# etzinis/sudo_rm_rf

Hardware: NVIDIA H100
Metric: mixtures_per_sec_forward_4s_8kHz_2src (higher is better)
Workload: dtype f32

## Files before the change

### sudo_rm_rf_b200/csrc/pointwise_mma.cu

```cuda
#include <cstdio>
#include <cstdlib>
#include <cstring>
#include <mutex>
#include <vector>
#include <cuda.h>
#include <cuda_bf16.h>
#include "common.cuh"

namespace sdr {

constexpr int kTileM = 128;
constexpr int kTileN = 128;
constexpr int kBlockK = 64;
constexpr int kStages = 3;
constexpr int kRawStages = 2;
constexpr int kBoxL = 32;
constexpr int kBoxBytes = 64 * kBoxL * 4;
constexpr int kRawStageBytes = kTileM / kBoxL * kBoxBytes;
constexpr int kBHalf = kTileN * 128;
constexpr int kBStageBytes = 2 * kBHalf;
constexpr int kSlotBytes = 2 * kBoxBytes;
constexpr int kSlots = 4;
constexpr int kConsWarps = 8, kTmaWarp = 8, kRawWarp = 9, kGatherWarps = 2;
template <bool WINDOW> constexpr int kMmaThreads = 32 * (kRawWarp + (WINDOW ? kGatherWarps : 1));

struct MmaArgs {
    const float* x;
    NormIn nin;
    const float* bias;
    int gate_channels;
    float* y;
    double* stats_out;
    int M, K, L;
    int l_tiles, n_tiles;
    int num_tiles;
    int epilogue;
    int win_k;
    int win_hop, win_pad, win_a;
    long long win_T;
};

__device__ __forceinline__ uint32_t smem_u32(const void* p) {
    return static_cast<uint32_t>(__cvta_generic_to_shared(p));
}
__device__ __forceinline__ void mbar_init(uint64_t* bar, uint32_t count) {
    asm volatile("mbarrier.init.shared::cta.b64 [%0], %1;" ::"r"(smem_u32(bar)), "r"(count) : "memory");
}
__device__ __forceinline__ void mbar_arrive(uint64_t* bar) {
    asm volatile("mbarrier.arrive.shared::cta.b64 _, [%0];" ::"r"(smem_u32(bar)) : "memory");
}
__device__ __forceinline__ void mbar_arrive_expect_tx(uint64_t* bar, uint32_t bytes) {
    asm volatile("mbarrier.arrive.expect_tx.shared::cta.b64 _, [%0], %1;" ::"r"(smem_u32(bar)), "r"(bytes) : "memory");
}
__device__ __forceinline__ void mbar_wait(uint64_t* bar, uint32_t parity) {
    const uint32_t addr = smem_u32(bar);
    uint32_t done;
    do {
        asm volatile(
            "{\n\t.reg .pred p;\n\t"
            "mbarrier.try_wait.parity.shared::cta.b64 p, [%1], %2;\n\t"
            "selp.u32 %0, 1, 0, p;\n\t}"
            : "=r"(done) : "r"(addr), "r"(parity) : "memory");
    } while (!done);
}
__device__ __forceinline__ void fence_barrier_init() {
    asm volatile("fence.mbarrier_init.release.cluster;" ::: "memory");
}
__device__ __forceinline__ void fence_proxy_async_smem() {
    asm volatile("fence.proxy.async.shared::cta;" ::: "memory");
}
__device__ __forceinline__ void tma_load_2d(void* smem_dst, const CUtensorMap* tm, uint64_t* bar, int c0, int c1) {
    asm volatile("cp.async.bulk.tensor.2d.shared::cluster.global.tile.mbarrier::complete_tx::bytes [%0], [%1, {%3, %4}], [%2];"
                 ::"r"(smem_u32(smem_dst)), "l"(tm), "r"(smem_u32(bar)), "r"(c0), "r"(c1) : "memory");
}
__device__ __forceinline__ void tma_load_3d(void* smem_dst, const CUtensorMap* tm, uint64_t* bar, int c0, int c1, int c2) {
    asm volatile("cp.async.bulk.tensor.3d.shared::cluster.global.tile.mbarrier::complete_tx::bytes [%0], [%1, {%3, %4, %5}], [%2];"
                 ::"r"(smem_u32(smem_dst)), "l"(tm), "r"(smem_u32(bar)), "r"(c0), "r"(c1), "r"(c2) : "memory");
}
__device__ __forceinline__ void tma_store_3d(const CUtensorMap* tm, const void* smem_src, int c0, int c1, int c2) {
    asm volatile("cp.async.bulk.tensor.3d.global.shared::cta.bulk_group [%0, {%2, %3, %4}], [%1];"
                 ::"l"(tm), "r"(smem_u32(smem_src)), "r"(c0), "r"(c1), "r"(c2) : "memory");
}
__device__ __forceinline__ void bulk_commit() { asm volatile("cp.async.bulk.commit_group;" ::: "memory"); }
__device__ __forceinline__ void bulk_wait_read_all() { asm volatile("cp.async.bulk.wait_group.read 0;" ::: "memory"); }
__device__ __forceinline__ void bulk_wait_all() { asm volatile("cp.async.bulk.wait_group 0;" ::: "memory"); }
__device__ __forceinline__ void named_bar_sync(uint32_t id, uint32_t threads) {
    asm volatile("bar.sync %0, %1;" ::"r"(id), "r"(threads) : "memory");
}

__device__ __forceinline__ uint64_t gmma_desc_sw128(uint32_t saddr, uint32_t lbo, uint32_t sbo) {
    uint64_t d = 0;
    d |= (uint64_t)((saddr >> 4) & 0x3FFF);
    d |= (uint64_t)((lbo >> 4) & 0x3FFF) << 16;
    d |= (uint64_t)((sbo >> 4) & 0x3FFF) << 32;
    d |= (uint64_t)1 << 62;
    return d;
}
constexpr uint32_t kBLbo = 16, kBSbo = 1024;

__device__ __forceinline__ void wgmma_fence() { asm volatile("wgmma.fence.sync.aligned;" ::: "memory"); }
__device__ __forceinline__ void wgmma_commit() { asm volatile("wgmma.commit_group.sync.aligned;" ::: "memory"); }
template <int N>
__device__ __forceinline__ void wgmma_wait() { asm volatile("wgmma.wait_group.sync.aligned %0;" ::"n"(N) : "memory"); }
__device__ __forceinline__ void wgmma_bf16_m64n128_rs(float (&d)[64], const uint32_t (&a)[4], uint64_t bdesc,
                                                      uint32_t accumulate) {
    asm volatile(
        "{\n\t.reg .pred p;\n\t"
        "setp.ne.b32 p, %69, 0;\n\t"
        "wgmma.mma_async.sync.aligned.m64n128k16.f32.bf16.bf16 "
        "{%0, %1, %2, %3, %4, %5, %6, %7, %8, %9, %10, %11, %12, %13, %14, %15, %16, %17, %18, %19, %20, %21, %22, "
        "%23, %24, %25, %26, %27, %28, %29, %30, %31, %32, %33, %34, %35, %36, %37, %38, %39, %40, %41, %42, %43, %44, "
        "%45, %46, %47, %48, %49, %50, %51, %52, %53, %54, %55, %56, %57, %58, %59, %60, %61, %62, %63}, "
        "{%64, %65, %66, %67}, %68, p, 1, 1, 0;\n\t}"
        : "+f"(d[0]), "+f"(d[1]), "+f"(d[2]), "+f"(d[3]), "+f"(d[4]), "+f"(d[5]), "+f"(d[6]), "+f"(d[7]),
          "+f"(d[8]), "+f"(d[9]), "+f"(d[10]), "+f"(d[11]), "+f"(d[12]), "+f"(d[13]), "+f"(d[14]), "+f"(d[15]),
          "+f"(d[16]), "+f"(d[17]), "+f"(d[18]), "+f"(d[19]), "+f"(d[20]), "+f"(d[21]), "+f"(d[22]), "+f"(d[23]),
          "+f"(d[24]), "+f"(d[25]), "+f"(d[26]), "+f"(d[27]), "+f"(d[28]), "+f"(d[29]), "+f"(d[30]), "+f"(d[31]),
          "+f"(d[32]), "+f"(d[33]), "+f"(d[34]), "+f"(d[35]), "+f"(d[36]), "+f"(d[37]), "+f"(d[38]), "+f"(d[39]),
          "+f"(d[40]), "+f"(d[41]), "+f"(d[42]), "+f"(d[43]), "+f"(d[44]), "+f"(d[45]), "+f"(d[46]), "+f"(d[47]),
          "+f"(d[48]), "+f"(d[49]), "+f"(d[50]), "+f"(d[51]), "+f"(d[52]), "+f"(d[53]), "+f"(d[54]), "+f"(d[55]),
          "+f"(d[56]), "+f"(d[57]), "+f"(d[58]), "+f"(d[59]), "+f"(d[60]), "+f"(d[61]), "+f"(d[62]), "+f"(d[63])
        : "r"(a[0]), "r"(a[1]), "r"(a[2]), "r"(a[3]), "l"(bdesc), "r"(accumulate)
        : "memory");
}

__global__ void pack_weight_mma_kernel(const float* __restrict__ W, uint8_t* __restrict__ out,
                                       int M, int Mpad, int Kreal, int K) {
    const long long i = (long long)blockIdx.x * blockDim.x + threadIdx.x;
    const long long chunks = (long long)Mpad * K / 8;
    if (i >= chunks) return;
    const int kc = (int)(i % (K / 8));
    const int m = (int)(i / (K / 8));
    const int kb = kc / 8, c = kc % 8;
    const int nt = m / kTileN, r = m % kTileN;
    const int KB = K / kBlockK;
    uint8_t* img = out + ((size_t)nt * KB + kb) * kBStageBytes;
    const size_t off = (size_t)(r >> 3) * 1024 + (size_t)(r & 7) * 128 + (size_t)((c ^ (r & 7)) << 4);
    __nv_bfloat16 hi[8], lo[8];
#pragma unroll
    for (int e = 0; e < 8; ++e) {
        const int k = kc * 8 + e;
        const float v = (m < M && k < Kreal) ? W[(size_t)m * Kreal + k] : 0.f;
        hi[e] = __float2bfloat16_rn(v);
        lo[e] = __float2bfloat16_rn(v - __bfloat162float(hi[e]));
    }
    *reinterpret_cast<uint4*>(img + off) = *reinterpret_cast<const uint4*>(hi);
    *reinterpret_cast<uint4*>(img + kBHalf + off) = *reinterpret_cast<const uint4*>(lo);
}

struct TileCoord { int sample, l0, n0; };
__device__ __forceinline__ TileCoord decode_tile(const MmaArgs& a, int tile) {
    TileCoord t;
    const int pos = tile / a.n_tiles;
    t.n0 = (tile - pos * a.n_tiles) * kTileN;
    t.sample = pos / a.l_tiles;
    t.l0 = (pos - t.sample * a.l_tiles) * kTileM;
    return t;
}

constexpr int kGroupSteps = 2;
constexpr int kGroups = kBlockK / 16 / kGroupSteps;
static_assert(kGroups == 2, "group g of every k-block uses fragment buffer g");
struct AFrag { uint32_t hi[kGroupSteps][4], lo[kGroupSteps][4]; };

template <bool WINDOW, int ACT, int MODE, bool STATS>
__global__ void __launch_bounds__(kMmaThreads<WINDOW>, 1)
pw_mma_kernel(const MmaArgs a, const __grid_constant__ CUtensorMap wmap,
              const __grid_constant__ CUtensorMap xmap,
              const __grid_constant__ CUtensorMap emap,
              const __grid_constant__ CUtensorMap ymap) {
    static_assert(!(WINDOW && ACT != 0), "the encoder's window operand has no activation");
    extern __shared__ uint8_t smem_raw[];
    uint8_t* smem = smem_raw + ((1024u - (smem_u32(smem_raw) & 1023u)) & 1023u);
    uint8_t* r_base = smem;
    uint8_t* b_base = r_base + kRawStages * kRawStageBytes;
    uint8_t* slots = b_base + kStages * kBStageBytes;
    float2* s_ab = reinterpret_cast<float2*>(slots + kSlots * kSlotBytes);
    float* s_sl = reinterpret_cast<float*>(s_ab + kRawStages * kBlockK);
    uint64_t* bars = reinterpret_cast<uint64_t*>(s_sl + kRawStages * kBlockK);
    uint64_t* full_bar = bars;
    uint64_t* empty_bar = full_bar + kStages;
    uint64_t* rfull_bar = empty_bar + kStages;
    uint64_t* rempty_bar = rfull_bar + kRawStages;
    uint64_t* slot_bar = rempty_bar + kRawStages;

    const int tid = threadIdx.x;
    const int warp = tid >> 5, lane = tid & 31;
    const int KB = a.K / kBlockK;
    const int tile0 = (int)blockIdx.x;
    const int tstep = (int)gridDim.x;

    if (warp == kTmaWarp && lane == 0) {
        for (int s = 0; s < kStages; ++s) { mbar_init(&full_bar[s], 1); mbar_init(&empty_bar[s], kConsWarps); }
        for (int s = 0; s < kRawStages; ++s) {
            mbar_init(&rfull_bar[s], WINDOW ? kGatherWarps : 2);
            mbar_init(&rempty_bar[s], kConsWarps);
        }
        for (int s = 0; s < kSlots; ++s) mbar_init(&slot_bar[s], 1);
        fence_barrier_init();
    }
    __syncthreads();

    if (warp >= kRawWarp) {
        int rs = 0;
        uint32_t rphase = 0;
        if constexpr (WINDOW) {
            constexpr int kGatherCh = kBlockK / kGatherWarps;
            const int c0 = (warp - kRawWarp) * kGatherCh;
#pragma unroll 1
            for (int tile = tile0; tile < a.num_tiles; tile += tstep) {
                const TileCoord tc = decode_tile(a, tile);
#pragma unroll 1
                for (int kb = 0; kb < KB; ++kb) {
                    uint8_t* rp = r_base + (size_t)rs * kRawStageBytes + (lane & 3) * 4;
#pragma unroll
                    for (int i0 = 0; i0 < kGatherCh; i0 += 16) {
                        float v[16][kTileM / kBoxL];
#pragma unroll
                        for (int i = 0; i < 16; ++i) {
                            const int k = kb * kBlockK + c0 + i0 + i;
                            const int ch = k / a.win_k, j = k - ch * a.win_k;
                            const float* src = a.x + ((size_t)tc.sample * a.win_a + ch) * a.win_T;
#pragma unroll
                            for (int b = 0; b < kTileM / kBoxL; ++b) {
                                const int l = tc.l0 + b * kBoxL + lane;
                                const long long t = (long long)a.win_hop * l + j - a.win_pad;
                                v[i][b] = (l < a.L && ch < a.win_a && t >= 0 && t < a.win_T) ? __ldg(src + t) : 0.f;
                            }
                        }
                        if (i0 == 0) mbar_wait(&rempty_bar[rs], rphase ^ 1);
#pragma unroll
                        for (int i = 0; i < 16; ++i) {
                            const int c = c0 + i0 + i;
#pragma unroll
                            for (int b = 0; b < kTileM / kBoxL; ++b)
                                *reinterpret_cast<float*>(rp + b * kBoxBytes + c * 128 + (((lane >> 2) ^ (c & 7)) << 4)) = v[i][b];
                        }
                    }
                    __syncwarp();
                    if (lane == 0) mbar_arrive(&rfull_bar[rs]);
                    if (++rs == kRawStages) { rs = 0; rphase ^= 1; }
                }
            }
        } else {
            const bool has_norm = a.nin.stats != nullptr;
            const double inv_count = 1.0 / a.nin.count;
#pragma unroll 1
            for (int tile = tile0; tile < a.num_tiles; tile += tstep) {
                const TileCoord tc = decode_tile(a, tile);
                float mean = 0.f, rstd = 1.f;
                if (has_norm) {
                    const double mu = a.nin.stats[2 * (size_t)tc.sample] * inv_count;
                    double var = a.nin.stats[2 * (size_t)tc.sample + 1] * inv_count - mu * mu;
                    var = var < 0.0 ? 0.0 : var;
                    mean = (float)mu;
                    rstd = rsqrtf((float)var + kGlnEps);
                }
#pragma unroll 1
                for (int kb = 0; kb < KB; ++kb) {
                    const int k = kb * kBlockK + 2 * lane;
                    float g[2] = {1.f, 1.f}, be[2] = {0.f, 0.f}, sl[2] = {1.f, 1.f};
                    if (has_norm) {
                        g[0] = __ldg(a.nin.gamma + k); g[1] = __ldg(a.nin.gamma + k + 1);
                        be[0] = __ldg(a.nin.beta + k); be[1] = __ldg(a.nin.beta + k + 1);
                    }
                    if constexpr (ACT == 2) { sl[0] = __ldg(a.nin.prelu + k); sl[1] = __ldg(a.nin.prelu + k + 1); }
                    mbar_wait(&rempty_bar[rs], rphase ^ 1);
                    if (lane == 0) {
                        mbar_arrive_expect_tx(&rfull_bar[rs], kRawStageBytes);
                        for (int b = 0; b < kTileM / kBoxL; ++b)
                            tma_load_3d(r_base + (size_t)rs * kRawStageBytes + b * kBoxBytes, &xmap, &rfull_bar[rs],
                                        tc.l0 + b * kBoxL, kb * kBlockK, tc.sample);
                    }
                    float aa[2] = {1.f, 1.f}, bb[2] = {0.f, 0.f};
                    if (has_norm) {
#pragma unroll
                        for (int e = 0; e < 2; ++e) { aa[e] = g[e] * rstd; bb[e] = be[e] - mean * aa[e]; }
                    }
                    *reinterpret_cast<float4*>(s_ab + rs * kBlockK + 2 * lane) = make_float4(aa[0], bb[0], aa[1], bb[1]);
                    if constexpr (ACT == 2) *reinterpret_cast<float2*>(s_sl + rs * kBlockK + 2 * lane) = make_float2(sl[0], sl[1]);
                    __syncwarp();
                    if (lane == 0) mbar_arrive(&rfull_bar[rs]);
                    if (++rs == kRawStages) { rs = 0; rphase ^= 1; }
                }
            }
        }
    } else if (warp == kTmaWarp) {
        if (lane == 0) {
            int stage = 0;
            uint32_t phase = 0;
            for (int tile = tile0; tile < a.num_tiles; tile += tstep) {
                const int nt = tile % a.n_tiles;
                for (int kb = 0; kb < KB; ++kb) {
                    mbar_wait(&empty_bar[stage], phase ^ 1);
                    mbar_arrive_expect_tx(&full_bar[stage], kBStageBytes);
                    tma_load_2d(b_base + (size_t)stage * kBStageBytes, &wmap, &full_bar[stage], 0, (nt * KB + kb) * 2 * kTileN);
                    if (++stage == kStages) { stage = 0; phase ^= 1; }
                }
            }
        }
        __syncwarp();
    } else {
        const int wg = warp >> 2;
        const int wr = warp & 3;
        const int q = lane & 3;
        const bool issuer = (tid & 127) == 0;
        const bool relu_out = WINDOW && a.epilogue == 2;
        const float slope = ACT == 1 ? __ldg(a.nin.prelu) : 1.f;
        const bool slope_le1 = slope <= 1.f;
        uint32_t boff[4];
#pragma unroll
        for (int v = 0; v < 4; ++v) {
            const uint32_t c = 2 * q + (v & 1), pp = 16 * (wr & 1) + (lane >> 2) + 8 * (v >> 1);
            boff[v] = c * 128 + (((pp >> 2) ^ c) << 4) + (pp & 3) * 4;
        }
        const uint32_t raw_box = (uint32_t)(2 * wg + (wr >> 1)) * kBoxBytes;
        uint8_t* const my_slots = slots + (size_t)(2 * wg) * kSlotBytes;
        auto fill_slot = [&](int tile, int h) {
            uint64_t* bar = &slot_bar[2 * wg + h];
            if constexpr (MODE == 0) {
                mbar_arrive(bar);
            } else {
                const TileCoord t = decode_tile(a, tile);
                const int c0 = t.l0 + 64 * wg;
                const int c1 = (MODE == 1 ? t.n0 : t.n0 % a.gate_channels) + 64 * h;
                uint8_t* const dst = my_slots + (size_t)h * kSlotBytes;
                mbar_arrive_expect_tx(bar, kSlotBytes);
                tma_load_3d(dst, &emap, bar, c0, c1, t.sample);
                tma_load_3d(dst + kBoxBytes, &emap, bar, c0 + kBoxL, c1, t.sample);
            }
        };
        if (issuer) { fill_slot(tile0, 0); fill_slot(tile0, 1); }

        int rs = 0, stage = 0, prev_stage = 0;
        uint32_t rphase = 0, phase = 0, slot_phase = 0;
        auto transform = [&](AFrag& f, int g) {
            if (g == 0) mbar_wait(&rfull_bar[rs], rphase);
            const uint8_t* rp = r_base + (size_t)rs * kRawStageBytes + raw_box;
            const float2* tab = s_ab + rs * kBlockK + 2 * q;
            const float* tsl = s_sl + rs * kBlockK + 2 * q;
#pragma unroll
            for (int s = 0; s < kGroupSteps; ++s) {
#pragma unroll
                for (int h = 0; h < 2; ++h) {
                    const int c = 16 * (g * kGroupSteps + s) + 8 * h;
                    float4 ab = make_float4(1.f, 0.f, 1.f, 0.f);
                    float2 sl = make_float2(1.f, 1.f);
                    if constexpr (!WINDOW) ab = *reinterpret_cast<const float4*>(tab + c);
                    if constexpr (ACT == 2) sl = *reinterpret_cast<const float2*>(tsl + c);
#pragma unroll
                    for (int ph = 0; ph < 2; ++ph) {
                        float y[2];
#pragma unroll
                        for (int e = 0; e < 2; ++e) {
                            const float x = *reinterpret_cast<const float*>(rp + boff[e + 2 * ph] + c * 128);
                            y[e] = WINDOW ? x : fmaf(x, e ? ab.z : ab.x, e ? ab.w : ab.y);
                            if constexpr (ACT == 1) {
                                const float t = y[e] * slope;
                                y[e] = slope_le1 ? fmaxf(y[e], t) : fminf(y[e], t);
                            } else if constexpr (ACT == 2) {
                                y[e] = y[e] >= 0.f ? y[e] : y[e] * (e ? sl.y : sl.x);
                            }
                        }
                        const uint32_t h0 = __float_as_uint(y[0]) & 0xffff0000u, h1 = __float_as_uint(y[1]) & 0xffff0000u;
                        const __nv_bfloat162 lo = __floats2bfloat162_rn(y[0] - __uint_as_float(h0), y[1] - __uint_as_float(h1));
                        f.hi[s][2 * h + ph] = __byte_perm(h0, h1, 0x7632);
                        f.lo[s][2 * h + ph] = *reinterpret_cast<const uint32_t*>(&lo);
                    }
                }
            }
            if (g == kGroups - 1) {
                __syncwarp();
                if (lane == 0) mbar_arrive(&rempty_bar[rs]);
                if (++rs == kRawStages) { rs = 0; rphase ^= 1; }
            }
        };
        float acc[64];
        auto mma_group = [&](int kb, int g, const AFrag& cur, AFrag& nxt) {
            if (g == 0) mbar_wait(&full_bar[stage], phase);
            const uint32_t sb_hi = smem_u32(b_base + (size_t)stage * kBStageBytes);
            const uint32_t sb_lo = sb_hi + kBHalf;
            wgmma_fence();
#pragma unroll
            for (int s = 0; s < kGroupSteps; ++s) {
                const int ks = g * kGroupSteps + s;
                const uint64_t dbh = gmma_desc_sw128(sb_hi + ks * 32, kBLbo, kBSbo);
                const uint64_t dbl = gmma_desc_sw128(sb_lo + ks * 32, kBLbo, kBSbo);
                wgmma_bf16_m64n128_rs(acc, cur.hi[s], dbh, (kb | ks) != 0 ? 1u : 0u);
                wgmma_bf16_m64n128_rs(acc, cur.lo[s], dbh, 1u);
                wgmma_bf16_m64n128_rs(acc, cur.hi[s], dbl, 1u);
            }
            wgmma_commit();
            wgmma_wait<1>();
            if (g == 0 && kb > 0) {
                __syncwarp();
                if (lane == 0) mbar_arrive(&empty_bar[prev_stage]);
            }
            if (g == kGroups - 1) {
                prev_stage = stage;
                if (++stage == kStages) { stage = 0; phase ^= 1; }
                if (kb + 1 < KB) transform(nxt, 0);
            } else {
                transform(nxt, g + 1);
            }
        };
        AFrag fa, fb;
#pragma unroll 1
        for (int tile = tile0; tile < a.num_tiles; tile += tstep) {
            const TileCoord tc = decode_tile(a, tile);
#pragma unroll
            for (int i = 0; i < 64; ++i) acc[i] = 0.f;
            transform(fa, 0);
#pragma unroll 1
            for (int kb = 0; kb < KB; ++kb) {
                mma_group(kb, 0, fa, fb);
                mma_group(kb, 1, fb, fa);
            }
            wgmma_wait<0>();
            __syncwarp();
            if (lane == 0) mbar_arrive(&empty_bar[prev_stage]);
            const int prem = a.L - (tc.l0 + wg * 64 + 32 * (wr >> 1) + 16 * (wr & 1) + (lane >> 2));
            StatAcc st;
            float rs_ = 0.f, rq = 0.f;
#pragma unroll
            for (int h = 0; h < 2; ++h) {
                uint8_t* const slot = my_slots + (size_t)h * kSlotBytes;
                uint8_t* const box = slot + (wr >> 1) * kBoxBytes;
                const int m0 = tc.n0 + 64 * h + 2 * q;
                const int mrem = a.M - m0;
                mbar_wait(&slot_bar[2 * wg + h], slot_phase);
#pragma unroll
                for (int j = 0; j < 8; ++j) {
                    float bv[2];
#pragma unroll
                    for (int b = 0; b < 2; ++b) bv[b] = (a.bias && 8 * j + b < mrem) ? __ldg(a.bias + m0 + 8 * j + b) : 0.f;
#pragma unroll
                    for (int v = 0; v < 4; ++v) {
                        const int u = 4 * j + v, i = 32 * h + u;
                        float* e = reinterpret_cast<float*>(box + boff[v] + 1024 * j);
                        float o = acc[i] + bv[v & 1];
                        if (MODE == 1) o += *e;
                        if (MODE == 2) o = fmaxf(o, 0.f) * *e;
                        if constexpr (WINDOW) { if (relu_out) o = fmaxf(o, 0.f); }
                        *e = o;
                        if (STATS && 8 * j + (v & 1) < mrem && 8 * (v >> 1) < prem) { rs_ += o; rq = fmaf(o, o, rq); }
                        if (STATS && (i & 15) == 15) { st.add_run(rs_, rq); rs_ = rq = 0.f; }
                    }
                }
                if constexpr (WINDOW) {
                    named_bar_sync(1 + wg, 128);
#pragma unroll 4
                    for (int r = wr; r < 64; r += 4) {
                        const int m = tc.n0 + 64 * h + r;
#pragma unroll
                        for (int half = 0; half < 2; ++half) {
                            const int p = tc.l0 + wg * 64 + half * kBoxL + lane;
                            const float v = *reinterpret_cast<const float*>(
                                slot + half * kBoxBytes + r * 128 + (((lane >> 2) ^ (r & 7)) << 4) + (lane & 3) * 4);
                            if (m < a.M && p < a.L) a.y[((size_t)tc.sample * a.M + m) * a.L + p] = v;
                        }
                    }
                    named_bar_sync(1 + wg, 128);
                } else {
                    fence_proxy_async_smem();
                    named_bar_sync(1 + wg, 128);
                    if (issuer) {
                        const int c0 = tc.l0 + wg * 64, c1 = tc.n0 + 64 * h;
                        tma_store_3d(&ymap, slot, c0, c1, tc.sample);
                        tma_store_3d(&ymap, slot + kBoxBytes, c0 + kBoxL, c1, tc.sample);
                        bulk_commit();
                        bulk_wait_read_all();
                    }
                }
                if (issuer && tile + tstep < a.num_tiles) fill_slot(tile + tstep, h);
            }
            slot_phase ^= 1;
            if (STATS) {
                const double ds = warp_sum_f64(st.s), dq = warp_sum_f64(st.q);
                if (lane == 0) {
                    atomicAdd(a.stats_out + 2 * (size_t)tc.sample, ds);
                    atomicAdd(a.stats_out + 2 * (size_t)tc.sample + 1, dq);
                }
            }
        }
        if (!WINDOW && issuer) bulk_wait_all();
    }
}

static inline int mma_pad_m(int M) { return (M + kTileN - 1) / kTileN * kTileN; }

bool pointwise_mma_eligible(int M, int K) {
    return M >= 32 && K >= kBlockK && (K % kBlockK) == 0;
}

size_t pointwise_mma_packed_bytes(int M, int K) {
    if (!pointwise_mma_eligible(M, K)) return 0;
    return (size_t)mma_pad_m(M) * K * 4;
}

int pack_pointwise_mma(const float* W, int M, int K, void* packed, cudaStream_t st) {
    if (!pointwise_mma_eligible(M, K)) return SDR_ERR_UNSUPPORTED;
    const int Mpad = mma_pad_m(M);
    const long long chunks = (long long)Mpad * K / 8;
    pack_weight_mma_kernel<<<(unsigned)((chunks + 255) / 256), 256, 0, st>>>(
        W, static_cast<uint8_t*>(packed), M, Mpad, K, K);
    return cudaGetLastError() == cudaSuccess ? SDR_OK : SDR_ERR_CUDA;
}

constexpr size_t kMmaSmemBytes = 1024 + (size_t)kRawStages * kRawStageBytes + (size_t)kStages * kBStageBytes +
                                 (size_t)kSlots * kSlotBytes + kRawStages * kBlockK * (sizeof(float2) + sizeof(float)) +
                                 (2 * kStages + 2 * kRawStages + kSlots) * sizeof(uint64_t);
static_assert(kMmaSmemBytes <= 232448, "exceeds the 227 KB a CTA may own on sm_90");

typedef CUresult (*EncodeTiledFn)(CUtensorMap*, CUtensorMapDataType, cuuint32_t, void*, const cuuint64_t*,
                                  const cuuint64_t*, const cuuint32_t*, const cuuint32_t*, CUtensorMapInterleave,
                                  CUtensorMapSwizzle, CUtensorMapL2promotion, CUtensorMapFloatOOBfill);
static EncodeTiledFn encode_tiled_fn() {
    static EncodeTiledFn fn = [] {
        void* ptr = nullptr;
        cudaDriverEntryPointQueryResult qres = cudaDriverEntryPointSymbolNotFound;
        if (cudaGetDriverEntryPoint("cuTensorMapEncodeTiled", &ptr, cudaEnableDefault, &qres) != cudaSuccess ||
            qres != cudaDriverEntryPointSuccess)
            ptr = nullptr;
        return reinterpret_cast<EncodeTiledFn>(ptr);
    }();
    return fn;
}

static int make_weight_map(CUtensorMap* tm, const void* wpk, size_t bytes) {
    memset(tm, 0, sizeof(*tm));
    EncodeTiledFn enc = encode_tiled_fn();
    if (!enc) return SDR_ERR_CUDA;
    const cuuint64_t dims[2] = {32, (cuuint64_t)(bytes / 128)};
    const cuuint64_t strides[1] = {128};
    const cuuint32_t box[2] = {32, (cuuint32_t)(2 * kTileN)};
    const cuuint32_t estr[2] = {1, 1};
    const CUresult r = enc(tm, CU_TENSOR_MAP_DATA_TYPE_FLOAT32, 2, const_cast<void*>(wpk), dims, strides, box, estr,
                           CU_TENSOR_MAP_INTERLEAVE_NONE, CU_TENSOR_MAP_SWIZZLE_NONE,
                           CU_TENSOR_MAP_L2_PROMOTION_L2_256B, CU_TENSOR_MAP_FLOAT_OOB_FILL_NONE);
    return r == CUDA_SUCCESS ? SDR_OK : SDR_ERR_UNSUPPORTED;
}

static int make_act_map(CUtensorMap* tm, const float* x, int samples, int C, int L) {
    memset(tm, 0, sizeof(*tm));
    EncodeTiledFn enc = encode_tiled_fn();
    if (!enc) return SDR_ERR_CUDA;
    const cuuint64_t dims[3] = {(cuuint64_t)L, (cuuint64_t)C, (cuuint64_t)samples};
    const cuuint64_t strides[2] = {(cuuint64_t)L * 4, (cuuint64_t)L * C * 4};
    const cuuint32_t box[3] = {(cuuint32_t)kBoxL, 64, 1};
    const cuuint32_t estr[3] = {1, 1, 1};
    const CUresult r = enc(tm, CU_TENSOR_MAP_DATA_TYPE_FLOAT32, 3, const_cast<float*>(x), dims, strides, box, estr,
                           CU_TENSOR_MAP_INTERLEAVE_NONE, CU_TENSOR_MAP_SWIZZLE_128B,
                           CU_TENSOR_MAP_L2_PROMOTION_L2_256B, CU_TENSOR_MAP_FLOAT_OOB_FILL_NONE);
    return r == CUDA_SUCCESS ? SDR_OK : SDR_ERR_UNSUPPORTED;
}
static_assert(kBlockK == 64 && kTileN == 2 * 64, "activation boxes are 64 channels: one k-block, half a channel tile");

struct MmaLaunchInfo { const void* fn; int dev; int sms; };
static std::mutex g_launch_mutex;
static std::vector<MmaLaunchInfo> g_launch_info;

template <bool WINDOW, typename Kern>
static int launch_persistent(Kern kern, const MmaArgs& a, const CUtensorMap& wmap, const CUtensorMap& xmap,
                             const CUtensorMap& emap, const CUtensorMap& ymap, cudaStream_t st) {
    int dev = 0;
    if (cudaGetDevice(&dev) != cudaSuccess) return SDR_ERR_CUDA;
    int sms = 0;
    {
        std::lock_guard<std::mutex> lock(g_launch_mutex);
        for (const MmaLaunchInfo& e : g_launch_info)
            if (e.fn == reinterpret_cast<const void*>(kern) && e.dev == dev) { sms = e.sms; break; }
        if (sms == 0) {
            if (cudaFuncSetAttribute(kern, cudaFuncAttributeMaxDynamicSharedMemorySize, (int)kMmaSmemBytes) != cudaSuccess) {
                cudaGetLastError();
                return SDR_ERR_CUDA;
            }
            if (cudaDeviceGetAttribute(&sms, cudaDevAttrMultiProcessorCount, dev) != cudaSuccess || sms <= 0) return SDR_ERR_CUDA;
            g_launch_info.push_back(MmaLaunchInfo{reinterpret_cast<const void*>(kern), dev, sms});
        }
    }
    const int grid = a.num_tiles < sms ? a.num_tiles : sms;
    kern<<<grid, kMmaThreads<WINDOW>, kMmaSmemBytes, st>>>(a, wmap, xmap, emap, ymap);
    if (cudaGetLastError() != cudaSuccess) return SDR_ERR_CUDA;
    return SDR_OK;
}

int launch_pointwise_mma(const float* x, const NormIn& nin, const void* wpk, const float* bias,
                         const float* residual, const float* gate, int gate_channels,
                         float* y, double* stats_out, int samples, int M, int K, int L,
                         int epilogue, cudaStream_t st) {
    auto misaligned = [](const float* p) { return (reinterpret_cast<uintptr_t>(p) % 16) != 0; };
    if (!pointwise_mma_eligible(M, K) || (L % 4) != 0 || misaligned(x) || misaligned(y) ||
        (epilogue != 1 && misaligned(residual)) || (epilogue == 1 && misaligned(gate)))
        return SDR_ERR_UNSUPPORTED;
    if (samples <= 0 || L <= 0 || !x || !wpk || !y) return SDR_ERR_BAD_ARGUMENT;
    if (epilogue == 1 && (!gate || gate_channels <= 0)) return SDR_ERR_BAD_ARGUMENT;
    if (epilogue == 1 && (gate_channels % kTileN) != 0) return SDR_ERR_UNSUPPORTED;
    if (reinterpret_cast<uintptr_t>(wpk) % 16) return SDR_ERR_BAD_ARGUMENT;
    MmaArgs a;
    a.x = x; a.nin = nin; a.bias = bias;
    a.gate_channels = gate_channels; a.y = y; a.stats_out = stats_out;
    a.M = M; a.K = K; a.L = L; a.epilogue = epilogue;
    a.win_k = 0; a.win_hop = 0; a.win_pad = 0; a.win_a = 0; a.win_T = 0;
    a.n_tiles = mma_pad_m(M) / kTileN;
    a.l_tiles = (L + kTileM - 1) / kTileM;
    const long long tiles = (long long)samples * a.l_tiles * a.n_tiles;
    if (tiles > 0x7fffffffLL) return SDR_ERR_UNSUPPORTED;
    a.num_tiles = (int)tiles;
    const int act = nin.prelu ? (nin.prelu_pc ? 2 : 1) : 0;
    const int mode = epilogue == 1 ? 2 : (residual ? 1 : 0);
    const bool stats = stats_out != nullptr;
    CUtensorMap wmap, xmap, emap, ymap;
    if (int rc = make_weight_map(&wmap, wpk, pointwise_mma_packed_bytes(M, K))) return rc;
    if (int rc = make_act_map(&xmap, x, samples, K, L)) return rc;
    if (int rc = make_act_map(&ymap, y, samples, M, L)) return rc;
    memset(&emap, 0, sizeof(emap));
    if (mode == 1)
        if (int rc = make_act_map(&emap, residual, samples, M, L)) return rc;
    if (mode == 2)
        if (int rc = make_act_map(&emap, gate, samples, gate_channels, L)) return rc;
#define SDR_MMA_CASE(A, MD, ST)                                                                                   \
    if (act == A && mode == MD && stats == ST)                                                                    \
        return launch_persistent<false>(pw_mma_kernel<false, A, MD, ST>, a, wmap, xmap, emap, ymap, st);
    SDR_MMA_CASE(0, 0, false) SDR_MMA_CASE(0, 0, true)
    SDR_MMA_CASE(1, 0, false) SDR_MMA_CASE(1, 0, true)
    SDR_MMA_CASE(0, 1, false) SDR_MMA_CASE(0, 1, true)
    SDR_MMA_CASE(1, 1, false) SDR_MMA_CASE(1, 1, true)
    SDR_MMA_CASE(0, 2, false) SDR_MMA_CASE(0, 2, true)
    SDR_MMA_CASE(1, 2, false) SDR_MMA_CASE(1, 2, true)
    SDR_MMA_CASE(2, 0, false) SDR_MMA_CASE(2, 0, true)
#undef SDR_MMA_CASE
    return SDR_ERR_UNSUPPORTED;
}

static inline int enc_kpad(int A, int Kk) { return (A * Kk + kBlockK - 1) / kBlockK * kBlockK; }

size_t encoder_mma_packed_bytes(int N, int A, int Kk) {
    if (N < 32 || A < 1 || Kk < 3) return 0;
    return (size_t)mma_pad_m(N) * enc_kpad(A, Kk) * 4;
}

int pack_encoder_mma(const float* W, int N, int A, int Kk, void* packed, cudaStream_t st) {
    if (!encoder_mma_packed_bytes(N, A, Kk)) return SDR_ERR_UNSUPPORTED;
    const int Mpad = mma_pad_m(N), K = enc_kpad(A, Kk);
    const long long chunks = (long long)Mpad * K / 8;
    pack_weight_mma_kernel<<<(unsigned)((chunks + 255) / 256), 256, 0, st>>>(
        W, static_cast<uint8_t*>(packed), N, Mpad, A * Kk, K);
    return cudaGetLastError() == cudaSuccess ? SDR_OK : SDR_ERR_CUDA;
}

int launch_encoder_mma(const float* wav, const void* wpk, const float* bias, int relu, float* enc, double* stats,
                       int B, int A, long long T, int N, int Kk, int L, int pad, cudaStream_t st) {
    if (!encoder_mma_packed_bytes(N, A, Kk)) return SDR_ERR_UNSUPPORTED;
    if (B <= 0 || T <= 0 || L <= 0 || !wav || !wpk || !enc) return SDR_ERR_BAD_ARGUMENT;
    MmaArgs a;
    a.x = wav; a.nin = NormIn{nullptr, nullptr, nullptr, nullptr, 1.0};
    a.bias = bias;
    a.gate_channels = 0; a.y = enc; a.stats_out = stats;
    a.M = N; a.K = enc_kpad(A, Kk); a.L = L; a.epilogue = relu ? 2 : 0;
    a.win_k = Kk; a.win_hop = Kk / 2; a.win_pad = pad; a.win_a = A; a.win_T = T;
    a.n_tiles = mma_pad_m(N) / kTileN;
    a.l_tiles = (L + kTileM - 1) / kTileM;
    const long long tiles = (long long)B * a.l_tiles * a.n_tiles;
    if (tiles > 0x7fffffffLL) return SDR_ERR_UNSUPPORTED;
    a.num_tiles = (int)tiles;
    CUtensorMap wmap, none;
    if (int rc = make_weight_map(&wmap, wpk, encoder_mma_packed_bytes(N, A, Kk))) return rc;
    memset(&none, 0, sizeof(none));
    if (stats) return launch_persistent<true>(pw_mma_kernel<true, 0, 0, true>, a, wmap, none, none, none, st);
    return launch_persistent<true>(pw_mma_kernel<true, 0, 0, false>, a, wmap, none, none, none, st);
}

}
```

Baseline: 2579.

## Move epilogue TMA stores and slot refills to a dedicated store warp

Adds a dedicated store warp for the non-window pointwise GEMM kernel. Consumer warpgroups now only arrive on a new per-slot full barrier, and the store warp issues the TMA stores, waits for the reads to finish, and refills the slot with residual or gate data for the next tile. This removes the named-barrier sync and the blocking bulk_wait_read from the consumer path, so math warps can move on to the next tile. The cost is one extra warp, extra mbarriers, and a single thread that serialises all four slots' stores and refills.

```diff
diff --git a/sudo_rm_rf_b200/csrc/pointwise_mma.cu b/sudo_rm_rf_b200/csrc/pointwise_mma.cu
--- a/sudo_rm_rf_b200/csrc/pointwise_mma.cu
+++ b/sudo_rm_rf_b200/csrc/pointwise_mma.cu
@@ -21,8 +21,9 @@
 constexpr int kBStageBytes = 2 * kBHalf;
 constexpr int kSlotBytes = 2 * kBoxBytes;
 constexpr int kSlots = 4;
-constexpr int kConsWarps = 8, kTmaWarp = 8, kRawWarp = 9, kGatherWarps = 2;
-template <bool WINDOW> constexpr int kMmaThreads = 32 * (kRawWarp + (WINDOW ? kGatherWarps : 1));
+constexpr int kConsWarps = 8, kTmaWarp = 8, kRawWarp = 9, kStoreWarp = 10, kGatherWarps = 2;
+constexpr int kMmaThreads = 32 * (kStoreWarp + 1);
+static_assert(kRawWarp + kGatherWarps == kStoreWarp + 1, "window mode's gather warps take the raw and store warps' places");
 
 struct MmaArgs {
     const float* x;
@@ -164,7 +165,7 @@
 struct AFrag { uint32_t hi[kGroupSteps][4], lo[kGroupSteps][4]; };
 
 template <bool WINDOW, int ACT, int MODE, bool STATS>
-__global__ void __launch_bounds__(kMmaThreads<WINDOW>, 1)
+__global__ void __launch_bounds__(kMmaThreads, 1)
 pw_mma_kernel(const MmaArgs a, const __grid_constant__ CUtensorMap wmap,
               const __grid_constant__ CUtensorMap xmap,
               const __grid_constant__ CUtensorMap emap,
@@ -183,6 +184,7 @@
     uint64_t* rfull_bar = empty_bar + kStages;
     uint64_t* rempty_bar = rfull_bar + kRawStages;
     uint64_t* slot_bar = rempty_bar + kRawStages;
+    uint64_t* slot_full = slot_bar + kSlots;
 
     const int tid = threadIdx.x;
     const int warp = tid >> 5, lane = tid & 31;
@@ -196,12 +198,12 @@
             mbar_init(&rfull_bar[s], WINDOW ? kGatherWarps : 2);
             mbar_init(&rempty_bar[s], kConsWarps);
         }
-        for (int s = 0; s < kSlots; ++s) mbar_init(&slot_bar[s], 1);
+        for (int s = 0; s < kSlots; ++s) { mbar_init(&slot_bar[s], 1); mbar_init(&slot_full[s], kConsWarps / 2); }
         fence_barrier_init();
     }
     __syncthreads();
 
-    if (warp >= kRawWarp) {
+    if (WINDOW ? warp >= kRawWarp : warp == kRawWarp) {
         int rs = 0;
         uint32_t rphase = 0;
         if constexpr (WINDOW) {
@@ -300,11 +302,49 @@
             }
         }
         __syncwarp();
+    } else if (warp == kStoreWarp) {
+        if constexpr (!WINDOW) {
+            if (lane == 0) {
+                auto fill_slot = [&](int tile, int s) {
+                    if constexpr (MODE == 0) {
+                        mbar_arrive(&slot_bar[s]);
+                    } else {
+                        const TileCoord t = decode_tile(a, tile);
+                        const int c0 = t.l0 + 64 * (s >> 1);
+                        const int c1 = (MODE == 1 ? t.n0 : t.n0 % a.gate_channels) + 64 * (s & 1);
+                        uint8_t* const dst = slots + (size_t)s * kSlotBytes;
+                        mbar_arrive_expect_tx(&slot_bar[s], kSlotBytes);
+                        tma_load_3d(dst, &emap, &slot_bar[s], c0, c1, t.sample);
+                        tma_load_3d(dst + kBoxBytes, &emap, &slot_bar[s], c0 + kBoxL, c1, t.sample);
+                    }
+                };
+                for (int s = 0; s < kSlots; ++s) fill_slot(tile0, s);
+                uint32_t phase = 0;
+#pragma unroll 1
+                for (int tile = tile0; tile < a.num_tiles; tile += tstep) {
+                    const TileCoord tc = decode_tile(a, tile);
+#pragma unroll 1
+                    for (int i = 0; i < kSlots; ++i) {
+                        const int h = i >> 1, wg = i & 1, s = 2 * wg + h;
+                        uint8_t* const slot = slots + (size_t)s * kSlotBytes;
+                        const int c0 = tc.l0 + 64 * wg, c1 = tc.n0 + 64 * h;
+                        mbar_wait(&slot_full[s], phase);
+                        tma_store_3d(&ymap, slot, c0, c1, tc.sample);
+                        tma_store_3d(&ymap, slot + kBoxBytes, c0 + kBoxL, c1, tc.sample);
+                        bulk_commit();
+                        bulk_wait_read_all();
+                        if (tile + tstep < a.num_tiles) fill_slot(tile + tstep, s);
+                    }
+                    phase ^= 1;
+                }
+                bulk_wait_all();
+            }
+            __syncwarp();
+        }
     } else {
         const int wg = warp >> 2;
         const int wr = warp & 3;
         const int q = lane & 3;
-        const bool issuer = (tid & 127) == 0;
         const bool relu_out = WINDOW && a.epilogue == 2;
         const float slope = ACT == 1 ? __ldg(a.nin.prelu) : 1.f;
         const bool slope_le1 = slope <= 1.f;
@@ -316,21 +356,6 @@
         }
         const uint32_t raw_box = (uint32_t)(2 * wg + (wr >> 1)) * kBoxBytes;
         uint8_t* const my_slots = slots + (size_t)(2 * wg) * kSlotBytes;
-        auto fill_slot = [&](int tile, int h) {
-            uint64_t* bar = &slot_bar[2 * wg + h];
-            if constexpr (MODE == 0) {
-                mbar_arrive(bar);
-            } else {
-                const TileCoord t = decode_tile(a, tile);
-                const int c0 = t.l0 + 64 * wg;
-                const int c1 = (MODE == 1 ? t.n0 : t.n0 % a.gate_channels) + 64 * h;
-                uint8_t* const dst = my_slots + (size_t)h * kSlotBytes;
-                mbar_arrive_expect_tx(bar, kSlotBytes);
-                tma_load_3d(dst, &emap, bar, c0, c1, t.sample);
-                tma_load_3d(dst + kBoxBytes, &emap, bar, c0 + kBoxL, c1, t.sample);
-            }
-        };
-        if (issuer) { fill_slot(tile0, 0); fill_slot(tile0, 1); }
 
         int rs = 0, stage = 0, prev_stage = 0;
         uint32_t rphase = 0, phase = 0, slot_phase = 0;
@@ -428,7 +453,7 @@
                 uint8_t* const box = slot + (wr >> 1) * kBoxBytes;
                 const int m0 = tc.n0 + 64 * h + 2 * q;
                 const int mrem = a.M - m0;
-                mbar_wait(&slot_bar[2 * wg + h], slot_phase);
+                if constexpr (!WINDOW) mbar_wait(&slot_bar[2 * wg + h], slot_phase);
 #pragma unroll
                 for (int j = 0; j < 8; ++j) {
                     float bv[2];
@@ -463,16 +488,9 @@
                     named_bar_sync(1 + wg, 128);
                 } else {
                     fence_proxy_async_smem();
-                    named_bar_sync(1 + wg, 128);
-                    if (issuer) {
-                        const int c0 = tc.l0 + wg * 64, c1 = tc.n0 + 64 * h;
-                        tma_store_3d(&ymap, slot, c0, c1, tc.sample);
-                        tma_store_3d(&ymap, slot + kBoxBytes, c0 + kBoxL, c1, tc.sample);
-                        bulk_commit();
-                        bulk_wait_read_all();
-                    }
-                }
-                if (issuer && tile + tstep < a.num_tiles) fill_slot(tile + tstep, h);
+                    __syncwarp();
+                    if (lane == 0) mbar_arrive(&slot_full[2 * wg + h]);
+                }
             }
             slot_phase ^= 1;
             if (STATS) {
@@ -483,7 +501,6 @@
                 }
             }
         }
-        if (!WINDOW && issuer) bulk_wait_all();
     }
 }
 
@@ -509,7 +526,7 @@
 
 constexpr size_t kMmaSmemBytes = 1024 + (size_t)kRawStages * kRawStageBytes + (size_t)kStages * kBStageBytes +
                                  (size_t)kSlots * kSlotBytes + kRawStages * kBlockK * (sizeof(float2) + sizeof(float)) +
-                                 (2 * kStages + 2 * kRawStages + kSlots) * sizeof(uint64_t);
+                                 (2 * kStages + 2 * kRawStages + 2 * kSlots) * sizeof(uint64_t);
 static_assert(kMmaSmemBytes <= 232448, "exceeds the 227 KB a CTA may own on sm_90");
 
 typedef CUresult (*EncodeTiledFn)(CUtensorMap*, CUtensorMapDataType, cuuint32_t, void*, const cuuint64_t*,
@@ -560,7 +577,7 @@
 static std::mutex g_launch_mutex;
 static std::vector<MmaLaunchInfo> g_launch_info;
 
-template <bool WINDOW, typename Kern>
+template <typename Kern>
 static int launch_persistent(Kern kern, const MmaArgs& a, const CUtensorMap& wmap, const CUtensorMap& xmap,
                              const CUtensorMap& emap, const CUtensorMap& ymap, cudaStream_t st) {
     int dev = 0;
@@ -580,7 +597,7 @@
         }
     }
     const int grid = a.num_tiles < sms ? a.num_tiles : sms;
-    kern<<<grid, kMmaThreads<WINDOW>, kMmaSmemBytes, st>>>(a, wmap, xmap, emap, ymap);
+    kern<<<grid, kMmaThreads, kMmaSmemBytes, st>>>(a, wmap, xmap, emap, ymap);
     if (cudaGetLastError() != cudaSuccess) return SDR_ERR_CUDA;
     return SDR_OK;
 }
@@ -621,7 +638,7 @@
         if (int rc = make_act_map(&emap, gate, samples, gate_channels, L)) return rc;
 #define SDR_MMA_CASE(A, MD, ST)                                                                                   \
     if (act == A && mode == MD && stats == ST)                                                                    \
-        return launch_persistent<false>(pw_mma_kernel<false, A, MD, ST>, a, wmap, xmap, emap, ymap, st);
+        return launch_persistent(pw_mma_kernel<false, A, MD, ST>, a, wmap, xmap, emap, ymap, st);
     SDR_MMA_CASE(0, 0, false) SDR_MMA_CASE(0, 0, true)
     SDR_MMA_CASE(1, 0, false) SDR_MMA_CASE(1, 0, true)
     SDR_MMA_CASE(0, 1, false) SDR_MMA_CASE(0, 1, true)
@@ -667,8 +684,8 @@
     CUtensorMap wmap, none;
     if (int rc = make_weight_map(&wmap, wpk, encoder_mma_packed_bytes(N, A, Kk))) return rc;
     memset(&none, 0, sizeof(none));
-    if (stats) return launch_persistent<true>(pw_mma_kernel<true, 0, 0, true>, a, wmap, none, none, none, st);
-    return launch_persistent<true>(pw_mma_kernel<true, 0, 0, false>, a, wmap, none, none, none, st);
-}
-
-}
+    if (stats) return launch_persistent(pw_mma_kernel<true, 0, 0, true>, a, wmap, none, none, none, st);
+    return launch_persistent(pw_mma_kernel<true, 0, 0, false>, a, wmap, none, none, none, st);
+}
+
+}
```

After: 2664, median of 6. +3.3%, better.
